# driskai/scenario_gym

Measured on NVIDIA B200. Metric: entity-steps/s, batched rollout+collision, higher is better.
Workload: dtype f64

## Files before the change

### scenario_gym_b200/csrc/sg_common.cuh

```cuda
#pragma once
#include <cuda_runtime.h>
#include <math.h>
#include <stdio.h>
#include <string.h>

#include "sg_device.cuh"
#include "sg_layout.h"

static __constant__ double c_ngon[64][2] = {
#include "sg_ngon.inc"
};

struct Grp {
  int n, s, M, G, W, H, QCAP, bar_id;
  unsigned mask;
  int64_t i, nm;
  double* corners;
  double* actbuf;
  double* rbox;
  unsigned corners_sh, rbox_sh;
  double* tcold;
  double* hcs;
  double* pedbuf;
  float4* pednb;
// ... 637 lines not shown
      group_sync(c);
    }
    const int swapped = *flag;
    ++round;
    if (!swapped) break;
  }
  if (r < c.M) c.posof[c.sid[r]] = (uint16_t)r;
}
SG_DEV void sorted_scatter(const Grp& c) {
  const int p = c.posof[c.s];
  const float k = c.skey[p];
  int np = p;
#pragma unroll
  for (int d = 1; d <= SG_SORT_WIN; ++d) {
    np -= c.skey[p - d] > k ? 1 : 0;
    np += c.skey[p + d] < k ? 1 : 0;
  }
  c.aabb[np] = c.tmpbox[c.s];
  c.sid[np] = (uint16_t)c.s;
  c.posof[c.s] = (uint16_t)np;
}
template <bool VERIFY = false>
SG_DEV void broad_phase_sorted(const Grp& c, int parity) {
  const int r = c.s;
  const float4 mb = c.aabb[r];
  if (VERIFY) {
    const float nx = c.aabb[r + 1].x;
    if (c.posof[c.sid[r]] != r || mb.x > nx) c.sflag[3] = 1;
  }
  if (!(mb.x <= mb.z)) return;
  const float4* nb = c.aabb + r + 1;
  int* acc = c.acc + parity * ACC_N;
  auto push = [&](int d) {
    const int q = atomicAdd(&acc[ACC_QCOUNT], 1);
    if (q < c.QCAP) c.queue[q] = ((uint32_t)c.sid[r] << 16) | (uint32_t)c.sid[r + d];
  };
  uint32_t hits = 0;
#pragma unroll
  for (int dd = 0; dd < SG_SWEEP_WIN; ++dd) {
    const float4 ob = nb[dd];
    SG_AABB_TEST(hits, mb, ob, 1u << dd);
  }
  while (hits) {
    const int dd = __ffs(hits) - 1;
    hits &= hits - 1;
    push(dd + 1);
  }
  for (int d = SG_SWEEP_WIN + 1; r + d < c.M && c.aabb[r + d].x <= mb.z; ++d) {
    const float4 ob = c.aabb[r + d];
    if (mb.x <= ob.z && ob.x <= mb.z && mb.y <= ob.w && ob.y <= mb.w) push(d);
  }
}

SG_DEV void publish_ego_box(const Grp& c) {
  const double eW = c.boxp[c.s], eL = c.boxp[c.G + c.s];
  c.egop[EGO_W] = eW; c.egop[EGO_L] = eL;
  c.egop[EGO_RHW] = 1.0 / (0.5 * eW); c.egop[EGO_RHL] = 1.0 / (0.5 * eL);
}

SG_DEV void unit_norm(double a, double b, double& nn, double& rn) {
  const double s2 = a * a + b * b, d = s2 - 1.0;
  if (fabs(d) < 1e-8) {
    nn = 1.0 + 0.5 * d;
    const double r0 = 2.0 - nn, e = __fma_rn(-nn, r0, 1.0);
    rn = __fma_rn(r0, e, r0);
  } else {
    nn = fast_sqrt(s2);
    rn = fast_rcp(nn);
  }
}

SG_DEV void publish_ego(const Grp& c, bool present, double x, double y, double ec, double es,
                        double vx, double vy) {
  double einv[2];
  {
    double nn, rn;
    unit_norm(es, ec, nn, rn);
    einv[0] = div_r(es, nn, rn);
    einv[1] = div_r(-ec, nn, rn);
  }
  double* E = c.egop;
  E[EGO_X] = x; E[EGO_Y] = y;
  E[EGO_C] = ec; E[EGO_S] = es;
  E[EGO_INV0] = einv[0]; E[EGO_INV1] = einv[1];
  const double hd[2] = {dot2(ec, es, einv[0], einv[1]), dot2(ec, es, ec, es)};
  E[EGO_HD0] = hd[0]; E[EGO_HD1] = hd[1];
  double hinv[2];
  {
    double nn, rn;
    unit_norm(hd[1], hd[0], nn, rn);
    hinv[0] = div_r(hd[1], nn, rn);
    hinv[1] = div_r(-hd[0], nn, rn);
  }
  E[EGO_HINV0] = hinv[0]; E[EGO_HINV1] = hinv[1];
  const double v0 = dot2(vx, vy, einv[0], einv[1]), v1 = dot2(vx, vy, ec, es);
  E[EGO_V0] = v0; E[EGO_V1] = v1;
  E[EGO_VNORM] = fnorm2(v0, v1);
  E[EGO_VLONG] = fabs(dot2(v0, v1, hd[0], hd[1]));
  E[EGO_PRESENT] = present ? 1.0 : 0.0;
}


SG_DEV double qx(unsigned qa, unsigned qs, int k) { return lds_f64(qa + 2u * (unsigned)(k & 3) * qs); }
SG_DEV double qy(unsigned qa, unsigned qs, int k) { return lds_f64(qa + (2u * (unsigned)(k & 3) + 1u) * qs); }
SG_DEV int quad_orientation_sh(unsigned qa, unsigned qs) {
  int s = orient_sign(qx(qa, qs, 0), qy(qa, qs, 0), qx(qa, qs, 1), qy(qa, qs, 1), qx(qa, qs, 2), qy(qa, qs, 2));
  if (s == 0)
    s = orient_sign(qx(qa, qs, 1), qy(qa, qs, 1), qx(qa, qs, 2), qy(qa, qs, 2), qx(qa, qs, 3), qy(qa, qs, 3));
  return s;
}

static __device__ __noinline__ bool line_hits_quad(unsigned qa, unsigned qs, double ax, double ay, double bx,
                                            double by) {
  int pos = 0, neg = 0;
#pragma unroll 1
  for (int m = 0; m < 4; ++m) {
    const int sg = orient_sign(ax, ay, bx, by, qx(qa, qs, m), qy(qa, qs, m));
    pos += sg > 0;
    neg += sg < 0;
  }
  return !(pos == 4 || neg == 4);
}

static __device__ __noinline__ bool quad_hits_centered_rect(unsigned qa, unsigned qs, double a, double b) {
  const int o = quad_orientation_sh(qa, qs);
#pragma unroll 1
  for (int k = 0; k < 4; ++k) {
    const double x0 = qx(qa, qs, k), y0 = qy(qa, qs, k), x1 = qx(qa, qs, k + 1), y1 = qy(qa, qs, k + 1);
    const double dx = x1 - x0, dy = y1 - y0;
    const double py = ((o > 0) == (dx > 0) || dx == 0) ? b : -b;
    const double px = ((o > 0) == (dy > 0) && dy != 0) ? -a : a;
    if (orient_sign(x0, y0, x1, y1, px, py) * o < 0) return false;
  }
  return true;
}

static __device__ __noinline__ bool quad_hits_hsegment(unsigned qa, unsigned qs, double w, double c) {
  const int o = quad_orientation_sh(qa, qs);
#pragma unroll 1
  for (int k = 0; k < 4; ++k) {
    const double x0 = qx(qa, qs, k), y0 = qy(qa, qs, k), x1 = qx(qa, qs, k + 1), y1 = qy(qa, qs, k + 1);
    if (orient_sign(x0, y0, x1, y1, -w, c) * o < 0 && orient_sign(x0, y0, x1, y1, w, c) * o < 0)
      return false;
  }
  return true;
}

static __device__ __noinline__ bool rss_box_hits_segment(unsigned qa, unsigned qs, double x0, double y0,
                                                  double x1, double y1) {
  const Quad q = load_quad_shared(qa, qs);
  return quad_intersects_segment(q, quad_orientation(q), x0, y0, x1, y1);
}

struct RssConst {
  double CLR, RT, MAXA, MINA, r2mina;
};

SG_DEV void rss_ratios(const Grp& c, double x, double y, double* out, int ost) {
  const double* E = c.egop;
  const double eh0 = E[EGO_C], eh1 = E[EGO_S], ei0 = E[EGO_INV0], ei1 = E[EGO_INV1];
  const double dirc = c.hcs[c.s], dirs = c.hcs[c.G + c.s];
  const double bw = c.boxp[c.s], bl = c.boxp[c.G + c.s];
  const double d0 = x - E[EGO_X], d1 = y - E[EGO_Y];
  const double pos0 = dot2(d0, d1, ei0, ei1), pos1 = dot2(d0, d1, eh0, eh1);
  const double hd0 = dot2(dirc, dirs, ei0, ei1), hd1 = dot2(dirc, dirs, eh0, eh1);
  const double eW = E[EGO_W], eL = E[EGO_L];
  const double hn = fnorm2(hd1, hd0), rhn = fast_rcp(hn);
  const double inv0 = div_r(hd1, hn, rhn), inv1 = div_r(-hd0, hn, rhn);
  const double wl_inv = fabs(dot2(bw, bl, inv0, inv1));
  const double wl_dir = fabs(dot2(bw, bl, hd0, hd1));
  const double actual_lat = py_max(1e-6, fabs(pos0) - 0.5 * eW - 0.5 * wl_inv);
  const double actual_long = py_max(1e-6, fabs(pos1) - 0.5 * eL - 0.5 * wl_dir);
  out[2 * ost] = fabs(div_r(actual_lat, 0.5 * eW, E[EGO_RHW]));
  out[3 * ost] = fabs(div_r(actual_long, 0.5 * eL, E[EGO_RHL]));
}

template <bool RATIOS = true>
SG_DEV int rss_hazard(const RssConst& K, const Grp& c, double x, double y, double vx, double vy,
                      uint8_t& state, double* out, int ost) {
  const double* E = c.egop;
  const double eh0 = E[EGO_C], eh1 = E[EGO_S], ei0 = E[EGO_INV0], ei1 = E[EGO_INV1];
  const double dirc = c.hcs[c.s], dirs = c.hcs[c.G + c.s];
  const double bw = c.boxp[c.s], bl = c.boxp[c.G + c.s];
  const double d0 = x - E[EGO_X], d1 = y - E[EGO_Y];
  const double pos0 = dot2(d0, d1, ei0, ei1), pos1 = dot2(d0, d1, eh0, eh1);
  const double hd0 = dot2(dirc, dirs, ei0, ei1), hd1 = dot2(dirc, dirs, eh0, eh1);
  const double v0 = dot2(vx, vy, ei0, ei1), v1 = dot2(vx, vy, eh0, eh1);
  const double eW = E[EGO_W], eL = E[EGO_L];
  const double eHD0 = E[EGO_HD0], eHD1 = E[EGO_HD1];
  double slong;
  {
    const double dp = dot2(eHD0, eHD1, hd0, hd1);
    const double a = fabs(K.MAXA * dp);
    const double hv = dot2(v0, v1, eHD0, eHD1);
    const double rta = K.RT * a;
    const bool ahead = 0.0 > pos1;
    const double vf = ahead ? E[EGO_VNORM] : hv, vr = ahead ? hv : E[EGO_VNORM];
    const double a2 = 2 * a;
    const double vf2a = div_r(vf * vf, a2, fast_rcp(a2));
    const double u = vr + rta;
    const double dd_s = py_max(0, vr * K.RT + py_min(vf2a, 0.5 * a * (K.RT * K.RT)) +
                                      div_r(u * u, 2 * K.MINA, K.r2mina) - vf2a);
    const double v1e = E[EGO_VLONG], av2 = fabs(hv);
    const double u1 = v1e + rta, u2 = av2 + rta;
    const double dd_o = py_max(0, (2 * v1e + rta) * K.RT / 2 + div_r(u1 * u1, 2 * K.MINA, K.r2mina) +
                                      (2 * av2 + rta) * K.RT / 2 + div_r(u2 * u2, 2 * K.MINA, K.r2mina));
    const bool same = dp > 0;
    const bool early = same ? (vr == 0.0) : (np_sign(pos1) == np_sign(v1));
    const double dd = same ? dd_s : dd_o;
    slong = fabs(early ? K.CLR + 0.5 * eL : dd + K.CLR + 0.5 * eL);
  }
  double slat;
  {
    const double k = fabs(dot2(E[EGO_HINV0], E[EGO_HINV1], hd0, hd1));
    const double amax = K.MAXA * k, amin = K.MINA * k;
    const double v = fabs(v0);
    const double den = 2 * amin, rden = fast_rcp(den);
    const double w = K.RT * amax, u = v + w;
    const double dl = py_max(0, 0.5 * K.RT * (2 * v + w) + div_r(u * u, den, rden) -
                                    0.5 * (K.RT * K.RT) * amax - div_r(w * w, den, rden));
    const bool conv = np_sign(-pos0) == np_sign(v0);
    const bool early = conv && v == 0.0;
    const double dd = (conv && !early) ? dl : 0.0;
    slat = fabs(early ? K.CLR + 0.5 * eW : dd + K.CLR + 0.5 * eW);
  }
  out[0] = slat;
  out[ost] = slong;
  if (RATIOS) {
    const double hn = fnorm2(hd1, hd0), rhn = fast_rcp(hn);
    const double inv0 = div_r(hd1, hn, rhn), inv1 = div_r(-hd0, hn, rhn);
    const double wl_inv = fabs(dot2(bw, bl, inv0, inv1));
    const double wl_dir = fabs(dot2(bw, bl, hd0, hd1));
    const double actual_lat = py_max(1e-6, fabs(pos0) - 0.5 * eW - 0.5 * wl_inv);
    const double actual_long = py_max(1e-6, fabs(pos1) - 0.5 * eL - 0.5 * wl_dir);
    out[2 * ost] = fabs(div_r(actual_lat, 0.5 * eW, E[EGO_RHW]));
    out[3 * ost] = fabs(div_r(actual_long, 0.5 * eL, E[EGO_RHL]));
  }
  if ((state >> 2) & 3) return SG_RSS_FOUND;
  double box[8];
#pragma unroll
  for (int q = 0; q < 4; ++q) {
    const double c0 = c.corners[(2 * q) * c.G + c.s] - E[EGO_X];
    const double c1 = c.corners[(2 * q + 1) * c.G + c.s] - E[EGO_Y];
    box[2 * q] = dot2(c0, c1, ei0, ei1);
    box[2 * q + 1] = dot2(c0, c1, eh0, eh1);
  }
  double* rbp = c.rbox + c.s;
#pragma unroll
  for (int q = 0; q < 8; ++q) rbp[q * c.G] = box[q];
  const unsigned rb = c.rbox_sh + (unsigned)c.s * 8u, st = (unsigned)c.G * 8u;
  const double bxmin = min2(min2(box[0], box[2]), min2(box[4], box[6]));
  const double bxmax = max2(max2(box[0], box[2]), max2(box[4], box[6]));
  const double bymin = min2(min2(box[1], box[3]), min2(box[5], box[7]));
  const double bymax = max2(max2(box[1], box[3]), max2(box[5], box[7]));
  bool inter = false;
  if (!(bxmin > slat || bxmax < -slat || bymin > slong || bymax < -slong)) {
    bool corner_in = false;
#pragma unroll
    for (int q = 0; q < 4; ++q)
      corner_in = corner_in || (fabs(box[2 * q]) <= slat && fabs(box[2 * q + 1]) <= slong);
    inter = corner_in || quad_hits_centered_rect(rb, st, slat, slong);
  }
  if (inter) {
    const int marker = state & 3;
    if (marker == 1) { state |= 2 << 2; return SG_RSS_UNSAFE_LONGITUDINAL; }
    if (marker == 2) { state |= 1 << 2; return SG_RSS_UNSAFE_LATERAL; }
    const double ed[2] = {eW, eL};
    double inv[2];
    inverse_direction(ed, inv);
    const double lhs = fabs(fabs(pos0) - fabs(dot2(pos0, pos1, ed[0], ed[1]))) / slat;
    const double rhs = fabs(fabs(pos1 - dot2(pos0, pos1, inv[0], inv[1])) / slong);
    if (lhs > rhs) { state |= 2 << 2; return SG_RSS_UNSAFE_LONGITUDINAL; }
    state |= 1 << 2;
    return SG_RSS_UNSAFE_LATERAL;
  }
  const double L100 = 100 * slong, W100 = 100 * slat;
  bool lat = false, lon = false;
  if (!(bxmin > slat || bxmax < -slat || bymin > L100 || bymax < -L100)) {
    if (bymax < L100 && bymin > -L100) {
      int pos1 = 0, neg1 = 0, pos2 = 0, neg2 = 0;
      bool unsure = false;
#pragma unroll
      for (int q = 0; q < 4; ++q) {
        const double pp = L100 * box[2 * q], rr = slat * box[2 * q + 1];
        const double d1 = pp - rr, d2 = pp + rr, tol = 4e-16 * (fabs(pp) + fabs(rr));
        unsure = unsure || !(fabs(d1) > tol) || !(fabs(d2) > tol);
        pos1 += d1 > 0; neg1 += d1 < 0;
        pos2 += d2 > 0; neg2 += d2 < 0;
      }
      if (unsure)
        lat = line_hits_quad(rb, st, slat, L100, -slat, 100 * -slong) ||
              line_hits_quad(rb, st, -slat, L100, slat, 100 * -slong);
      else
        lat = !(pos1 == 4 || neg1 == 4) || !(pos2 == 4 || neg2 == 4);
    } else
      lat = rss_box_hits_segment(rb, st, slat, L100, -slat, 100 * -slong) ||
            rss_box_hits_segment(rb, st, -slat, L100, slat, 100 * -slong);
  }
  if (!(bxmin > W100 || bxmax < -W100)) {
    if (bxmin > -W100 && bxmax < W100) {
      lon = (bymin <= slong && slong <= bymax) || (bymin <= -slong && -slong <= bymax);
    } else {
      if (!(bymin > slong || bymax < slong)) lon = quad_hits_hsegment(rb, st, W100, slong);
      if (!lon && !(bymin > -slong || bymax < -slong)) lon = quad_hits_hsegment(rb, st, W100, -slong);
    }
  }
  if (lat && lon) return SG_RSS_BOTH;
  if (lat) { state = (uint8_t)((state & ~3) | 1); return SG_RSS_LATERAL; }
  if (lon) { state = (uint8_t)((state & ~3) | 2); return SG_RSS_LONGITUDINAL; }
  return SG_RSS_SAFE;
}

#ifdef SG_FLAT_BOXES
static __device__ __noinline__ bool flat_pair_meets(unsigned pa, unsigned pb, unsigned qs) {
#pragma unroll 1
  for (int i = 0; i < 4; ++i) {
    const double ax = qx(pa, qs, i), ay = qy(pa, qs, i), bx = qx(pa, qs, i + 1), by = qy(pa, qs, i + 1);
#pragma unroll 1
    for (int j = 0; j < 4; ++j)
      if (segments_meet(ax, ay, bx, by, qx(pb, qs, j), qy(pb, qs, j), qx(pb, qs, j + 1), qy(pb, qs, j + 1))) return true;
  }
  return false;
}
#endif

static __device__ __noinline__ bool pair_collides(unsigned csh, const int8_t* orient, int G, int a, int b) {
  const unsigned qs = (unsigned)G * 8u;
  unsigned pa = csh + (unsigned)a * 8u, pb = csh + (unsigned)b * 8u;
  bool same = true;
#pragma unroll 1
  for (unsigned f = 0; f < 8; ++f) same = same && (lds_f64(pa + f * qs) == lds_f64(pb + f * qs));
  if (same) return false;
  int oa = orient[a], ob = orient[b];
#ifdef SG_FLAT_BOXES
  if (oa == 0 && ob == 0) return flat_pair_meets(pa, pb, qs);
#endif
#pragma unroll 1
  for (int pass = 0; pass < 2; ++pass) {
#pragma unroll 1
    for (int k = 0; k < 4; ++k) {
      const double ax = qx(pa, qs, k), ay = qy(pa, qs, k), bx = qx(pa, qs, k + 1), by = qy(pa, qs, k + 1);
      bool sep = true;
#ifdef SG_FLAT_BOXES
      int want = -oa;
#pragma unroll 1
      for (int m = 0; m < 4 && sep; ++m) {
        const int sg = orient_sign(ax, ay, bx, by, qx(pb, qs, m), qy(pb, qs, m));
        if (want == 0) want = sg;
        sep = sg != 0 && sg == want;
      }
#else
#pragma unroll 1
      for (int m = 0; m < 4 && sep; ++m)
        sep = orient_sign(ax, ay, bx, by, qx(pb, qs, m), qy(pb, qs, m)) * oa < 0;
#endif
      if (sep) return false;
    }
    const unsigned tp = pa; pa = pb; pb = tp;
    const int to = oa; oa = ob; ob = to;
  }
  return true;
}

struct PairSink {
  int* acc;
  uint32_t* bits;
  uint32_t* ego_now;
  uint32_t* rows;
  int W, ego_slot, first_slot;
};
SG_DEV PairSink make_sink(int features, uint32_t* coll_mask, const Grp& c, int ego_slot, int first_slot,
                          int parity) {
  PairSink k;
  k.acc = c.acc + parity * ACC_N;
  k.bits = c.bits + parity * c.W;
  k.ego_now = c.ego_now;
  k.rows = (features & SG_FEAT_COLL_MATRIX) ? coll_mask + (int64_t)c.n * c.M * c.W : nullptr;
  k.W = c.W; k.ego_slot = ego_slot; k.first_slot = first_slot;
  return k;
}

static __device__ __noinline__ void commit_pair(PairSink k, int a, int b) {
  const int lo = min(a, b), hi = max(a, b);
  atomicAdd(&k.acc[ACC_NPAIRS], 1);
  atomicMin(&k.acc[ACC_FIRST_PAIR], (lo << 16) | hi);
  if (lo == k.first_slot || hi == k.first_slot) k.acc[ACC_FIRST_HIT] = 1;
  atomicOr(&k.bits[lo >> 5], 1u << (lo & 31));
  atomicOr(&k.bits[hi >> 5], 1u << (hi & 31));
  if (lo == k.ego_slot) atomicOr(&k.ego_now[hi >> 5], 1u << (hi & 31));
  if (hi == k.ego_slot) atomicOr(&k.ego_now[lo >> 5], 1u << (lo & 31));
  if (k.rows) {
    atomicOr(&k.rows[(int64_t)lo * k.W + (hi >> 5)], 1u << (hi & 31));
    atomicOr(&k.rows[(int64_t)hi * k.W + (lo >> 5)], 1u << (lo & 31));
  }
}

SG_DEV int sat_classify(const double* A, const double* B) {
  const double e1ax = A[2] - A[0], e1ay = A[3] - A[1], e2ax = A[0] - A[6], e2ay = A[1] - A[7];
  const double e1bx = B[2] - B[0], e1by = B[3] - B[1], e2bx = B[0] - B[6], e2by = B[1] - B[7];
  const double dx = (B[0] + B[4]) - (A[0] + A[4]), dy = (B[1] + B[5]) - (A[1] + A[5]);
  const double scale = fabs(A[0]) + fabs(A[1]) + fabs(B[0]) + fabs(B[1]) + fabs(e1ax) + fabs(e1ay) + fabs(e2ax) +
                       fabs(e2ay) + fabs(e1bx) + fabs(e1by) + fabs(e2bx) + fabs(e2by);
  const double rel = 1e-9 * scale;
  bool apart = false, inside = true;
#define SG_SAT_AXIS(ax, ay)                                                                             \
  {                                                                                                     \
    const double gap = fabs(dx * (ax) + dy * (ay)) -                                                    \
                       (fabs(e1ax * (ax) + e1ay * (ay)) + fabs(e2ax * (ax) + e2ay * (ay)) +             \
                        fabs(e1bx * (ax) + e1by * (ay)) + fabs(e2bx * (ax) + e2by * (ay)));             \
    const double tol = rel * (fabs(ax) + fabs(ay));                                                     \
    apart = apart || gap > tol;                                                                         \
    inside = inside && gap < -tol;                                                                      \
  }
  SG_SAT_AXIS(e1ax, e1ay)
  SG_SAT_AXIS(e2ax, e2ay)
  SG_SAT_AXIS(e1bx, e1by)
  SG_SAT_AXIS(e2bx, e2by)
#undef SG_SAT_AXIS
  if (!(fabs(dx) + fabs(dy) > rel)) return 0;
  return apart ? -1 : (inside ? 1 : 0);
}

struct Obb {
  double cx, cy, ux, uy, vx, vy;
};
SG_DEV int sat_classify_obb(const Obb& A, const Obb& B) {
  const double dx = B.cx - A.cx, dy = B.cy - A.cy;
  const double scale = fabs(A.cx) + fabs(A.cy) + fabs(B.cx) + fabs(B.cy) + fabs(A.ux) + fabs(A.uy) + fabs(A.vx) +
                       fabs(A.vy) + fabs(B.ux) + fabs(B.uy) + fabs(B.vx) + fabs(B.vy);
  const double rel = 1e-9 * scale;
  bool apart = false, inside = true;
#define SG_OBB_AXIS(ax, ay)                                                                              \
  {                                                                                                     \
    const double gap = fabs(dx * (ax) + dy * (ay)) -                                                    \
                       (fabs(A.ux * (ax) + A.uy * (ay)) + fabs(A.vx * (ax) + A.vy * (ay)) +             \
                        fabs(B.ux * (ax) + B.uy * (ay)) + fabs(B.vx * (ax) + B.vy * (ay)));             \
    const double tol = rel * (fabs(ax) + fabs(ay));                                                     \
    apart = apart || gap > tol;                                                                         \
    inside = inside && gap < -tol;                                                                      \
  }
  SG_OBB_AXIS(A.ux, A.uy)
  SG_OBB_AXIS(A.vx, A.vy)
  SG_OBB_AXIS(B.ux, B.uy)
  SG_OBB_AXIS(B.vx, B.vy)
#undef SG_OBB_AXIS
  if (!(fabs(dx) + fabs(dy) > rel)) return 0;
  return apart ? -1 : (inside ? 1 : 0);
}

SG_DEV void record_pair(const PairSink& k, unsigned corners_sh, const int8_t* orient, int G, int a, int b) {
  if (pair_collides(corners_sh, orient, G, a, b)) commit_pair(k, a, b);
}

static __device__ __noinline__ void decide_pair(PairSink k, const double* corners, unsigned corners_sh,
                                                const int8_t* orient, int G, int a, int b) {
  double qa[8], qb[8];
#pragma unroll
  for (int f = 0; f < 8; ++f) { qa[f] = corners[f * G + a]; qb[f] = corners[f * G + b]; }
  const int v = sat_classify(qa, qb);
// ... 231 lines not shown
```

### scenario_gym_b200/csrc/sg_vehicle.cuh

```cuda
#pragma once
#include "sg_common.cuh"
#include "sg_internal.h"
#include "sg_pcg.cuh"

SG_DEV void cp_async4(unsigned smem_addr, const void* gsrc) {
  asm volatile("cp.async.ca.shared.global [%0], [%1], 4;" ::"r"(smem_addr), "l"(gsrc) : "memory");
}

template <bool RSS, int MC>
struct VehLayout {
  static constexpr GroupLayout value = make_layout(MC > 0 ? MC : 64, false, RSS, true, false);
};
template <bool RSS, int MAXT, int MINB, bool SORTED, bool LEAN = false, int ACT = ACT_F64, int MC = 0>
__global__ void __launch_bounds__(MAXT, MINB)
sg_vehicle_kernel(SgScene sc, SgParams p, SgState st, SgInputs in, int n_ticks, GroupLayout Lrt, SgRngDev rng) {
  extern __shared__ __align__(16) unsigned char smem[];
  const GroupLayout L = MC > 0 ? VehLayout<RSS, MC>::value : Lrt;
  const int G = L.G, M = MC > 0 ? MC : sc.n_slots, W = L.W;
  const int gpb = blockDim.x / G;
  const int gl = threadIdx.x / G;
  const int s = threadIdx.x - gl * G;
  const int n = blockIdx.x * gpb + gl;
  if (gl >= gpb || n >= sc.n_scenarios) return;
  Grp c;
// ... 33 lines not shown
        tc[2 * G] = st.safe_ratio[i]; tc[3 * G] = st.safe_ratio[nm + i];
      }
    }
    if (s == 0) {
      double* U = c.cold_d;
      U[COLD_T0] = st.t[n]; U[COLD_PT0] = st.prev_t[n];
      U[COLD_LEN] = sc.length[n];
      const int64_t er = sc.traj_off[(int64_t)n * M + ego_slot];
      U[COLD_OX] = __ldg(sc.traj_rows + er * 7 + 1);
      U[COLD_OY] = __ldg(sc.traj_rows + er * 7 + 2);
      U[COLD_R2MINA] = 1.0 / (2 * p.rss_min_long_accel);
    }
  }
  int tick = st.tick[n];
  bool done = st.done[n] != 0;
  load_cold(st, c, n, s, W, ego_slot);
  if (RSS && s == ego_slot) publish_ego_box(c);
  if (SORTED) sorted_setup(c);
  int sort_round = 0;
  group_sync(c);

  int limit = n_ticks < 0 ? p.max_ticks : n_ticks;
  if (limit > in.n_action_ticks) limit = in.n_action_ticks;
  int parity = 0;
  const int tick0 = tick;
  double* ab = c.actbuf + s;
  const unsigned ab_sh = (unsigned)__cvta_generic_to_shared(ab);
  const double* act = in.actions + c.i;
  const float* act32 = in.actions_f32 + c.i;
  unsigned long long* rq = (unsigned long long*)c.actbuf + s;
  if (ACT == ACT_RNG) {
    if (live && limit > 0) {
#pragma unroll 1
      for (int cc = 0; cc < 2; ++cc) {
        const sg_u128 q = sg_rng_slot_state(rng, cc, c.i + (int64_t)sc.scenario_base * M);
        rq[(2 * cc) * G] = (unsigned long long)q;
        rq[(2 * cc + 1) * G] = (unsigned long long)(q >> 64);
      }
    }
  } else if (ACT == ACT_F32) {
    if (live && limit > 0 && (!done || in.step_done)) { cp_async4(ab_sh, act32); cp_async4(ab_sh + G * 8, act32 + c.nm); }
    cp_async_commit();
  } else {
    if (live && limit > 0 && (!done || in.step_done)) { cp_async8(ab_sh, act); cp_async8(ab_sh + G * 8, act + c.nm); }
    cp_async_commit();
  }

  double* const corners0 = c.corners;
  const unsigned corners_sh0 = c.corners_sh;
  for (int k = 0; k < limit && (!done || in.step_done); ++k) {
    if (LEAN && lag) {
      c.corners = corners0 + parity * 8 * G;
      c.corners_sh = corners_sh0 + (unsigned)(parity * 8 * G * 8);
    }
    const double* U = c.cold_d;
    const double t = U[COLD_T0 + parity];
    const double next_t = t + p.timestep;
    const double dt = next_t - t;
    if (ACT != ACT_RNG) cp_async_wait_all();
    if (live && present) {
      double a_in, s_in;
      if (ACT == ACT_RNG) {
        const sg_u128 A = sg_u128_make(rng.a_hi, rng.a_lo), Cc = sg_u128_make(rng.c_hi, rng.c_lo);
        unsigned long long lo = rq[0], hi = rq[G];
        a_in = rng.low[0] + rng.scale[0] * sg_pcg_double(hi, lo);
        sg_u128 q = A * sg_u128_make(hi, lo) + Cc;
        rq[0] = (unsigned long long)q; rq[G] = (unsigned long long)(q >> 64);
        lo = rq[2 * G]; hi = rq[3 * G];
        s_in = rng.low[1] + rng.scale[1] * sg_pcg_double(hi, lo);
        q = A * sg_u128_make(hi, lo) + Cc;
        rq[2 * G] = (unsigned long long)q; rq[3 * G] = (unsigned long long)(q >> 64);
      } else if (ACT == ACT_F32) {
        a_in = (double)*(const float*)(ab + parity * 2 * G);
        s_in = (double)*(const float*)(ab + parity * 2 * G + G);
      } else {
        a_in = ab[parity * 2 * G];
        s_in = ab[parity * 2 * G + G];
      }
      const double accel = clipd(a_in, -p.veh_max_accel, p.veh_max_accel);
      const double steer = clipd(s_in, -p.veh_max_steer, p.veh_max_steer);
      const double dx = speed * cs, dy = speed * sn;
      const double tn = fabs(steer) <= 0.78 ? tan_small(steer) : tan_lib(steer);
      const double dh = div_r(speed * tn, c.boxp[G + s], tc[5 * G]);
      const double nx = x + dx * dt, ny = y + dy * dt, nh = h + dh * dt;
      double ns = speed + accel * dt;
      if (!p.veh_allow_reverse) ns = ns < 0.0 ? 0.0 : ns;
      if (p.veh_max_speed == p.veh_max_speed) ns = ns > p.veh_max_speed ? p.veh_max_speed : ns;
      speed = ns;
      const double rdt = fast_rcp(dt);
      const double ex = nx - x, ey = ny - y;
      vx = div_r(ex, dt, rdt); vy = div_r(ey, dt, rdt);
      tc[4 * G] = div_r(nh - h, dt, rdt);
      dist += fnorm2(ex, ey);
      x = nx; y = ny; h = nh;
      sincos_fast(h, sn, cs);
    }
    if (ACT == ACT_F64) {
      if (live && k + 1 < limit) {
        act += 2 * c.nm;
        cp_async8(ab_sh + (parity ^ 1) * 2 * G * 8, act);
        cp_async8(ab_sh + ((parity ^ 1) * 2 * G + G) * 8, act + c.nm);
      }
      cp_async_commit();
    } else if (ACT == ACT_F32) {
      if (live && k + 1 < limit) {
        act32 += 2 * c.nm;
        cp_async4(ab_sh + (parity ^ 1) * 2 * G * 8, act32);
        cp_async4(ab_sh + ((parity ^ 1) * 2 * G + G) * 8, act32 + c.nm);
      }
      cp_async_commit();
    }
    tick += 1;
    if (!LEAN && st.trace_cap > 0 && tick < st.trace_cap && s < M) {
      const int64_t i = c.i, nm = c.nm;
      st.trace_present[(int64_t)tick * nm + i] = present;
      double* tp = st.trace_pose + (int64_t)tick * 6 * nm + i;
      tp[0] = x; tp[nm] = y; tp[2 * nm] = st.pose[2 * nm + i]; tp[3 * nm] = h;
      tp[4 * nm] = st.pose[4 * nm + i]; tp[5 * nm] = st.pose[5 * nm + i];
      if (s == 0) st.trace_t[(int64_t)tick * sc.n_scenarios + n] = next_t;
    }
    if (s < M) {
      if (need_coll || feat_rss)
        publish_box<RSS, SORTED>(c, present, x, y, cs, sn, orient_hint, U[COLD_OX], U[COLD_OY]);
      if (!LEAN && matrix) {
        uint32_t* row = st.coll_mask + ((int64_t)n * M + s) * W;
        for (int w = 0; w < W; ++w) row[w] = 0;
      }
    }
    if (RSS && feat_rss && s == ego_slot) publish_ego(c, present, x, y, cs, sn, vx, vy);
    if (s == 0) {
      c.cold_d[COLD_T0 + (parity ^ 1)] = next_t;
      c.cold_d[COLD_PT0 + (parity ^ 1)] = t;
    }
    group_sync(c);
    bool resort = false;
    if (SORTED && need_coll) {
      resort = c.sflag[3] != 0;
      if (!resort) {
        if (s < M) sorted_scatter(c);
        group_sync(c);
      }
    }
    if (LEAN && lag && k > 0)
      lagged_epilogue(p, st, c, n + sc.scenario_base, s, W, G, ego_slot, parity ^ 1, tick - 1, t);
    if (live && present) {
      if (RSS && feat_rss) {
        rss_last = SG_RSS_NONE;
        rss_evald = false;
        if (next_t != 0.0 && s != ego_slot && c.egop[EGO_PRESENT] != 0.0) {
          RssConst KR;
          KR.CLR = p.rss_min_safe_clearance; KR.RT = p.rss_response_time;
          KR.MAXA = p.rss_max_long_accel; KR.MINA = p.rss_min_long_accel;
          KR.r2mina = c.cold_d[COLD_R2MINA];
          rss_last = (uint8_t)rss_hazard<!LEAN>(KR, c, x, y, vx, vy, rss_state, tc, G);
          rss_evald = true;
          const int found = (rss_state >> 2) & 3;
          if (found) atomicOr(&c.acc[parity * ACC_N + ACC_RSS], found == 2 ? 1 : 2);
        }
      }
      if (need_coll && !SORTED) broad_phase(c, parity);
    }
    if (SORTED && need_coll && !resort && s < M) broad_phase_sorted<true>(c, parity);
    group_sync(c);
    if (SORTED && need_coll && (resort || c.sflag[3] != 0)) {
      group_sync(c);
      if (s == 0) { c.sflag[3] = 0; c.acc[parity * ACC_N + ACC_QCOUNT] = 0; }
      if (s < M) { c.aabb[s] = c.tmpbox[s]; c.sid[s] = (uint16_t)s; }
      group_sync(c);
      sort_positions(c, sort_round);
      group_sync(c);
      if (s < M) broad_phase_sorted<false>(c, parity);
      group_sync(c);
    }
    if (LEAN && lag) {
      narrow_phase_lagged(p, st, c, s, G, ego_slot, first_slot, parity, live && present);
      if (c.acc[parity * ACC_N + ACC_QCOUNT] > c.QCAP) group_sync(c);
      const double ta = c.cold_d[COLD_T0 + (parity ^ 1)], dta = ta - c.cold_d[COLD_PT0 + (parity ^ 1)];
      done = (p.terminal & SG_TERM_MAX_LENGTH) && (ta + dta > c.cold_d[COLD_LEN]);
      if (s == ego_slot && (p.features & SG_FEAT_EGO_METRICS)) {
        double* m = c.cold_d;
        const double sp = fast_sqrt(vx * vx + vy * vy);
        const double w = ta > 0.0 ? div_r(m[COLD_AVG_T], ta, fast_rcp(ta)) : m[COLD_AVG_T] / ta;
        m[COLD_AVG] += (1.0 - w) * (sp - m[COLD_AVG]);
        m[COLD_AVG_T] = ta;
        m[COLD_MAX] = fmax(sp, m[COLD_MAX]);
        m[COLD_EGOD] = dist;
      }
    } else {
      done = finish_tick<true>(p, st, c, n + sc.scenario_base, s, W, G, ego_slot, first_slot, parity, tick,
                         c.cold_d[COLD_T0 + (parity ^ 1)], c.cold_d[COLD_T0 + (parity ^ 1)] - c.cold_d[COLD_PT0 + (parity ^ 1)],
                         c.cold_d[COLD_LEN], live, live && present, collided, vx, vy, 0.0, dist);
    }
    parity ^= 1;
  }
  if (LEAN && lag && tick > tick0) {
    group_sync(c);
    lagged_epilogue(p, st, c, n + sc.scenario_base, s, W, G, ego_slot, parity ^ 1, tick, c.cold_d[COLD_T0 + parity]);
    if (live && ((c.bits[s >> 5] >> (s & 31)) & 1)) collided = 1;
  }

  if (RSS && LEAN && live && present && rss_evald) rss_ratios(c, x, y, tc, G);
  if (live) {
    const int64_t i = c.i, nm = c.nm;
    st.pose[i] = x; st.pose[nm + i] = y; st.pose[3 * nm + i] = h;
    st.vel[i] = vx; st.vel[nm + i] = vy; st.vel[3 * nm + i] = tc[4 * G];
    if (tick > tick0 && present) { st.vel[2 * nm + i] = 0.0; st.vel[4 * nm + i] = 0.0; st.vel[5 * nm + i] = 0.0; }
    st.dist[i] = dist;
    st.speed[i] = speed;
    st.collided[i] = collided;
    if (RSS) {
      st.rss_state[i] = rss_state; st.rss_last[i] = rss_last;
      st.safe_dist[i] = tc[0]; st.safe_dist[nm + i] = tc[G];
      st.safe_ratio[i] = tc[2 * G]; st.safe_ratio[nm + i] = tc[3 * G];
    }
  }
  if (s == 0) {
    st.t[n] = c.cold_d[COLD_T0 + parity]; st.prev_t[n] = c.cold_d[COLD_PT0 + parity];
    st.tick[n] = tick; st.done[n] = done;
  }
  store_cold(st, c, n, s, W, ego_slot);
}

template <bool RSS>
static cudaError_t launch_vehicle_t(int n_scen, cudaStream_t s, const SgScene& sc, const SgParams& p,
                                    const SgState& st, const SgInputs& in, const SgRngDev& rng, int act,
                                    int n_ticks, const GroupLayout& L) {
  void (*kern)(SgScene, SgParams, SgState, SgInputs, int, GroupLayout, SgRngDev);
  int threads;
  const bool lean = sgi_vehicle_lean(p, st);
  if (!lean && act != ACT_F64) return cudaErrorNotSupported;
#define SG_VEH_PICK(T, B, S)                                                                   \
  (!lean ? sg_vehicle_kernel<RSS, T, B, S, false, ACT_F64>                                     \
         : act == ACT_RNG ? sg_vehicle_kernel<RSS, T, B, S, true, ACT_RNG>                     \
         : act == ACT_F32 ? sg_vehicle_kernel<RSS, T, B, S, true, ACT_F32>                     \
                          : sg_vehicle_kernel<RSS, T, B, S, true, ACT_F64>)
#define SG_VEH_PICK_M(T, B, S, MC_)                                                            \
  (act == ACT_RNG ? sg_vehicle_kernel<RSS, T, B, S, true, ACT_RNG, MC_>                        \
                  : sg_vehicle_kernel<RSS, T, B, S, true, ACT_F64, MC_>)
  const int M = sc.n_slots;
  const bool spec = lean && (act == ACT_RNG || act == ACT_F64);
  if (L.G <= SG_VEH_THREADS) {
    kern = (spec && M == 64) ? SG_VEH_PICK_M(SG_VEH_THREADS, SG_VEH_MINB, false, 64)
         : (spec && M == 128) ? SG_VEH_PICK_M(SG_VEH_THREADS, SG_VEH_MINB, false, 128)
                              : SG_VEH_PICK(SG_VEH_THREADS, SG_VEH_MINB, false);
    threads = SG_VEH_THREADS;
  } else if (L.G <= SG_THREADS) {
    kern = (spec && M == 256 && L.sorted) ? SG_VEH_PICK_M(SG_THREADS, 2, true, 256)
         : L.sorted ? SG_VEH_PICK(SG_THREADS, 2, true) : SG_VEH_PICK(SG_THREADS, 2, false);
    threads = SG_THREADS;
  }
  else { kern = L.sorted ? SG_VEH_PICK(1024, 1, true) : SG_VEH_PICK(1024, 1, false); threads = L.G; }
#undef SG_VEH_PICK
#undef SG_VEH_PICK_M
  const int gpb = threads / L.G;
  const int blocks = (n_scen + gpb - 1) / gpb;
  const size_t smem = (size_t)gpb * L.bytes;
  if (smem > 48 * 1024) {
    cudaError_t err = cudaFuncSetAttribute(kern, cudaFuncAttributeMaxDynamicSharedMemorySize, (int)smem);
    if (err != cudaSuccess) return err;
  }
  kern<<<blocks, threads, smem, s>>>(sc, p, st, in, n_ticks, L, rng);
  return cudaGetLastError();
}
```

Baseline: 17.22 billion.

## Add analytic separating-axis fast path for RSS geometry with noinline fallback

For the sorted vehicle kernel, the RSS hazard check first tries a closed-form separating-axis test on the oriented box against the safety rectangle and the lateral and longitudinal bands, with tolerance margins. It falls back to an out-of-line geometry stage that computes the rotated box in shared memory and flags which exact tests to run. The non-sorted path also gains an interval pre-test before the per-corner sign loop. The aim is to cut per-entity arithmetic, register pressure and divergence in RSS evaluation, at the cost of a noinline call on the fallback and a possible mismatch with the exact result near the tolerance edges.

```diff
diff --git a/scenario_gym_b200/csrc/sg_common.cuh b/scenario_gym_b200/csrc/sg_common.cuh
--- a/scenario_gym_b200/csrc/sg_common.cuh
+++ b/scenario_gym_b200/csrc/sg_common.cuh
@@ -813,6 +813,75 @@
   return quad_intersects_segment(q, quad_orientation(q), x0, y0, x1, y1);
 }
 
+enum : unsigned {
+  RSS_GEO_RECT = 1u,
+  RSS_GEO_LINES = 2u,
+  RSS_GEO_SEGS = 4u,
+  RSS_GEO_HSEG_P = 8u,
+  RSS_GEO_HSEG_M = 16u,
+  RSS_GEO_LAT = 32u,
+  RSS_GEO_LON = 64u,
+  RSS_GEO_INTER = 128u,
+};
+static __device__ __noinline__ unsigned rss_geometry_stage(unsigned ca, unsigned rb, unsigned st, unsigned ea,
+                                                           double slat, double slong) {
+  const double ex = lds_f64(ea + EGO_X * 8u), ey = lds_f64(ea + EGO_Y * 8u);
+  const double eh0 = lds_f64(ea + EGO_C * 8u), eh1 = lds_f64(ea + EGO_S * 8u);
+  const double ei0 = lds_f64(ea + EGO_INV0 * 8u), ei1 = lds_f64(ea + EGO_INV1 * 8u);
+  double* const box = (double*)__cvta_shared_to_generic(rb);
+  const unsigned G = st / 8u;
+  bool corner_in = false;
+#pragma unroll 1
+  for (unsigned q = 0; q < 4; ++q) {
+    const double c0 = lds_f64(ca + 2u * q * st) - ex;
+    const double c1 = lds_f64(ca + (2u * q + 1u) * st) - ey;
+    const double b0 = dot2(c0, c1, ei0, ei1), b1 = dot2(c0, c1, eh0, eh1);
+    box[2u * q * G] = b0;
+    box[(2u * q + 1u) * G] = b1;
+    corner_in = corner_in || (fabs(b0) <= slat && fabs(b1) <= slong);
+  }
+#define SG_BX(q) box[2u * (q) * G]
+#define SG_BY(q) box[(2u * (q) + 1u) * G]
+  const double bxmin = min2(min2(SG_BX(0), SG_BX(1)), min2(SG_BX(2), SG_BX(3)));
+  const double bxmax = max2(max2(SG_BX(0), SG_BX(1)), max2(SG_BX(2), SG_BX(3)));
+  const double bymin = min2(min2(SG_BY(0), SG_BY(1)), min2(SG_BY(2), SG_BY(3)));
+  const double bymax = max2(max2(SG_BY(0), SG_BY(1)), max2(SG_BY(2), SG_BY(3)));
+  const bool near = !(bxmin > slat || bxmax < -slat || bymin > slong || bymax < -slong);
+  if (near && corner_in) return RSS_GEO_INTER;
+  unsigned todo = near ? RSS_GEO_RECT : 0u;
+  {
+    const double L100 = 100 * slong, W100 = 100 * slat;
+    if (!(bxmin > slat || bxmax < -slat || bymin > L100 || bymax < -L100)) {
+      if (bymax < L100 && bymin > -L100) {
+        int pos1 = 0, neg1 = 0, pos2 = 0, neg2 = 0;
+        bool unsure = false;
+#pragma unroll 1
+        for (unsigned q = 0; q < 4; ++q) {
+          const double pp = L100 * SG_BX(q), rr = slat * SG_BY(q);
+          const double d1 = pp - rr, d2 = pp + rr, tol = 4e-16 * (fabs(pp) + fabs(rr));
+          unsure = unsure || !(fabs(d1) > tol) || !(fabs(d2) > tol);
+          pos1 += d1 > 0; neg1 += d1 < 0;
+          pos2 += d2 > 0; neg2 += d2 < 0;
+        }
+        if (unsure) todo |= RSS_GEO_LINES;
+        else if (!(pos1 == 4 || neg1 == 4) || !(pos2 == 4 || neg2 == 4)) todo |= RSS_GEO_LAT;
+      } else
+        todo |= RSS_GEO_SEGS;
+    }
+    if (!(bxmin > W100 || bxmax < -W100)) {
+      if (bxmin > -W100 && bxmax < W100) {
+        if ((bymin <= slong && slong <= bymax) || (bymin <= -slong && -slong <= bymax)) todo |= RSS_GEO_LON;
+      } else {
+        if (!(bymin > slong || bymax < slong)) todo |= RSS_GEO_HSEG_P;
+        if (!(bymin > -slong || bymax < -slong)) todo |= RSS_GEO_HSEG_M;
+      }
+    }
+  }
+#undef SG_BX
+#undef SG_BY
+  return todo;
+}
+
 struct RssConst {
   double CLR, RT, MAXA, MINA, r2mina;
 };
@@ -836,7 +905,7 @@
   out[3 * ost] = fabs(div_r(actual_long, 0.5 * eL, E[EGO_RHL]));
 }
 
-template <bool RATIOS = true>
+template <bool RATIOS = true, bool BAND = false>
 SG_DEV int rss_hazard(const RssConst& K, const Grp& c, double x, double y, double vx, double vy,
                       uint8_t& state, double* out, int ost) {
   const double* E = c.egop;
@@ -898,31 +967,141 @@
     out[3 * ost] = fabs(div_r(actual_long, 0.5 * eL, E[EGO_RHL]));
   }
   if ((state >> 2) & 3) return SG_RSS_FOUND;
-  double box[8];
+  if (!BAND) {
+    double box[8];
 #pragma unroll
-  for (int q = 0; q < 4; ++q) {
-    const double c0 = c.corners[(2 * q) * c.G + c.s] - E[EGO_X];
-    const double c1 = c.corners[(2 * q + 1) * c.G + c.s] - E[EGO_Y];
-    box[2 * q] = dot2(c0, c1, ei0, ei1);
-    box[2 * q + 1] = dot2(c0, c1, eh0, eh1);
-  }
-  double* rbp = c.rbox + c.s;
+    for (int q = 0; q < 4; ++q) {
+      const double c0 = c.corners[(2 * q) * c.G + c.s] - E[EGO_X];
+      const double c1 = c.corners[(2 * q + 1) * c.G + c.s] - E[EGO_Y];
+      box[2 * q] = dot2(c0, c1, ei0, ei1);
+      box[2 * q + 1] = dot2(c0, c1, eh0, eh1);
+    }
+    double* rbp = c.rbox + c.s;
 #pragma unroll
-  for (int q = 0; q < 8; ++q) rbp[q * c.G] = box[q];
-  const unsigned rb = c.rbox_sh + (unsigned)c.s * 8u, st = (unsigned)c.G * 8u;
-  const double bxmin = min2(min2(box[0], box[2]), min2(box[4], box[6]));
-  const double bxmax = max2(max2(box[0], box[2]), max2(box[4], box[6]));
-  const double bymin = min2(min2(box[1], box[3]), min2(box[5], box[7]));
-  const double bymax = max2(max2(box[1], box[3]), max2(box[5], box[7]));
-  bool inter = false;
-  if (!(bxmin > slat || bxmax < -slat || bymin > slong || bymax < -slong)) {
-    bool corner_in = false;
+    for (int q = 0; q < 8; ++q) rbp[q * c.G] = box[q];
+    const unsigned rb = c.rbox_sh + (unsigned)c.s * 8u, st = (unsigned)c.G * 8u;
+    const double bxmin = min2(min2(box[0], box[2]), min2(box[4], box[6]));
+    const double bxmax = max2(max2(box[0], box[2]), max2(box[4], box[6]));
+    const double bymin = min2(min2(box[1], box[3]), min2(box[5], box[7]));
+    const double bymax = max2(max2(box[1], box[3]), max2(box[5], box[7]));
+    bool inter = false;
+    if (!(bxmin > slat || bxmax < -slat || bymin > slong || bymax < -slong)) {
+      bool corner_in = false;
 #pragma unroll
-    for (int q = 0; q < 4; ++q)
-      corner_in = corner_in || (fabs(box[2 * q]) <= slat && fabs(box[2 * q + 1]) <= slong);
-    inter = corner_in || quad_hits_centered_rect(rb, st, slat, slong);
-  }
-  if (inter) {
+      for (int q = 0; q < 4; ++q)
+        corner_in = corner_in || (fabs(box[2 * q]) <= slat && fabs(box[2 * q + 1]) <= slong);
+      inter = corner_in || quad_hits_centered_rect(rb, st, slat, slong);
+    }
+    if (inter) {
+      const int marker = state & 3;
+      if (marker == 1) { state |= 2 << 2; return SG_RSS_UNSAFE_LONGITUDINAL; }
+      if (marker == 2) { state |= 1 << 2; return SG_RSS_UNSAFE_LATERAL; }
+      const double ed[2] = {eW, eL};
+      double inv[2];
+      inverse_direction(ed, inv);
+      const double lhs = fabs(fabs(pos0) - fabs(dot2(pos0, pos1, ed[0], ed[1]))) / slat;
+      const double rhs = fabs(fabs(pos1 - dot2(pos0, pos1, inv[0], inv[1])) / slong);
+      if (lhs > rhs) { state |= 2 << 2; return SG_RSS_UNSAFE_LONGITUDINAL; }
+      state |= 1 << 2;
+      return SG_RSS_UNSAFE_LATERAL;
+    }
+    const double L100 = 100 * slong, W100 = 100 * slat;
+    bool lat = false, lon = false;
+    if (!(bxmin > slat || bxmax < -slat || bymin > L100 || bymax < -L100)) {
+      if (bymax < L100 && bymin > -L100) {
+        const double a0 = L100 * bxmin, a1 = L100 * bxmax, b0 = slat * bymin, b1 = slat * bymax;
+        const double tl = 4e-16 * ((fabs(a0) + fabs(a1)) + (fabs(b0) + fabs(b1)));
+        if (!((a0 - b1 > tl || a1 - b0 < -tl) && (a0 + b0 > tl || a1 + b1 < -tl))) {
+          int pos1 = 0, neg1 = 0, pos2 = 0, neg2 = 0;
+          bool unsure = false;
+#pragma unroll
+          for (int q = 0; q < 4; ++q) {
+            const double pp = L100 * box[2 * q], rr = slat * box[2 * q + 1];
+            const double d1 = pp - rr, d2 = pp + rr, tol = 4e-16 * (fabs(pp) + fabs(rr));
+            unsure = unsure || !(fabs(d1) > tol) || !(fabs(d2) > tol);
+            pos1 += d1 > 0; neg1 += d1 < 0;
+            pos2 += d2 > 0; neg2 += d2 < 0;
+          }
+          if (unsure)
+            lat = line_hits_quad(rb, st, slat, L100, -slat, 100 * -slong) ||
+                  line_hits_quad(rb, st, -slat, L100, slat, 100 * -slong);
+          else
+            lat = !(pos1 == 4 || neg1 == 4) || !(pos2 == 4 || neg2 == 4);
+        }
+      } else
+        lat = rss_box_hits_segment(rb, st, slat, L100, -slat, 100 * -slong) ||
+              rss_box_hits_segment(rb, st, -slat, L100, slat, 100 * -slong);
+    }
+    if (!(bxmin > W100 || bxmax < -W100)) {
+      if (bxmin > -W100 && bxmax < W100) {
+        lon = (bymin <= slong && slong <= bymax) || (bymin <= -slong && -slong <= bymax);
+      } else {
+        if (!(bymin > slong || bymax < slong)) lon = quad_hits_hsegment(rb, st, W100, slong);
+        if (!lon && !(bymin > -slong || bymax < -slong)) lon = quad_hits_hsegment(rb, st, W100, -slong);
+      }
+    }
+    if (lat && lon) return SG_RSS_BOTH;
+    if (lat) { state = (uint8_t)((state & ~3) | 1); return SG_RSS_LATERAL; }
+    if (lon) { state = (uint8_t)((state & ~3) | 2); return SG_RSS_LONGITUDINAL; }
+    return SG_RSS_SAFE;
+  }
+  unsigned geo = 8u;
+  const double bcx = c.boxp[2 * c.G + c.s], bcy = c.boxp[3 * c.G + c.s];
+  const double hl = 0.5 * fabs(bl), hw = 0.5 * fabs(bw);
+  const double ah0 = fabs(hd0), ah1 = fabs(hd1);
+  const double del = 1e-9 * (((fabs(x) + fabs(y)) + (fabs(E[EGO_X]) + fabs(E[EGO_Y]))) +
+                             ((fabs(bl) + fabs(bw)) + (fabs(bcx) + fabs(bcy))));
+  if (hl > del && hw > del && ah0 + ah1 < 1.5 && del > 1e-150 && slat > 1e-100 && slong > 1e-100 &&
+      del + slat + slong < 1e50) {
+    const double c0 = pos0 + (bcx * hd0 - bcy * hd1), c1 = pos1 + (bcx * hd1 + bcy * hd0);
+    const double ac0 = fabs(c0), ac1 = fabs(c1);
+    const double ex = hl * ah0 + hw * ah1, ey = hl * ah1 + hw * ah0;
+    const double gx = ac0 - (ex + slat), gy = ac1 - (ey + slong);
+    bool apart = gx > del || gy > del;
+    if (!apart) {
+      const double mh = del * (ah0 + ah1);
+      const double gu = fabs(hd0 * c0 + hd1 * c1) - (hl + (ah0 * slat + ah1 * slong));
+      const double gv = fabs(hd0 * c1 - hd1 * c0) - (hw + (ah1 * slat + ah0 * slong));
+      if (gx < -del && gy < -del && gu < -mh && gv < -mh) geo = 1u;
+      apart = gu > mh || gv > mh;
+    }
+    if (apart) {
+      const double L100 = 100 * slong, W100 = 100 * slat;
+      const double ml = del * (L100 + slat);
+      const double P = L100 * c0, Q = slat * c1;
+      const double ea = L100 * ex + slat * ey;
+      bool lat_t = false, lat_f = ac1 - ey - L100 > del || (fabs(P - Q) - ea > ml && fabs(P + Q) - ea > ml);
+      if (!lat_f) {
+        const double A = L100 * hd0, B = slat * hd1, C = L100 * hd1, D = slat * hd0;
+        const double g1 = fabs(P - Q) - (hl * fabs(A - B) + hw * fabs(C + D));
+        const double g2 = fabs(P + Q) - (hl * fabs(A + B) + hw * fabs(C - D));
+        lat_t = ac1 + ey - L100 < -del && (g1 < -ml || g2 < -ml);
+        lat_f = g1 > ml && g2 > ml;
+      }
+      const double gp = fabs(c1 - slong) - ey, gm = fabs(c1 + slong) - ey;
+      const bool lon_t = ac0 + ex - W100 < -del && (gp < -del || gm < -del);
+      const bool lon_f = ac0 - ex - W100 > del || (gp > del && gm > del);
+      if ((lat_t || lat_f) && (lon_t || lon_f)) geo = (lat_t ? 2u : 0u) | (lon_t ? 4u : 0u);
+    }
+  }
+  if (geo == 8u) {
+    const unsigned rb = c.rbox_sh + (unsigned)c.s * 8u, st = (unsigned)c.G * 8u;
+    const unsigned todo = rss_geometry_stage(c.corners_sh + (unsigned)c.s * 8u, rb, st,
+                                             (unsigned)__cvta_generic_to_shared(E), slat, slong);
+    if ((todo & RSS_GEO_INTER) || ((todo & RSS_GEO_RECT) && quad_hits_centered_rect(rb, st, slat, slong))) {
+      geo = 1u;
+    } else {
+      const double L100 = 100 * slong, W100 = 100 * slat;
+      const bool lat = (todo & RSS_GEO_LAT) ||
+                       ((todo & RSS_GEO_LINES) && (line_hits_quad(rb, st, slat, L100, -slat, 100 * -slong) ||
+                                                   line_hits_quad(rb, st, -slat, L100, slat, 100 * -slong))) ||
+                       ((todo & RSS_GEO_SEGS) && (rss_box_hits_segment(rb, st, slat, L100, -slat, 100 * -slong) ||
+                                                  rss_box_hits_segment(rb, st, -slat, L100, slat, 100 * -slong)));
+      const bool lon = (todo & RSS_GEO_LON) || ((todo & RSS_GEO_HSEG_P) && quad_hits_hsegment(rb, st, W100, slong)) ||
+                       ((todo & RSS_GEO_HSEG_M) && quad_hits_hsegment(rb, st, W100, -slong));
+      geo = (lat ? 2u : 0u) | (lon ? 4u : 0u);
+    }
+  }  if (geo & 1u) {
     const int marker = state & 3;
     if (marker == 1) { state |= 2 << 2; return SG_RSS_UNSAFE_LONGITUDINAL; }
     if (marker == 2) { state |= 1 << 2; return SG_RSS_UNSAFE_LATERAL; }
@@ -935,37 +1114,7 @@
     state |= 1 << 2;
     return SG_RSS_UNSAFE_LATERAL;
   }
-  const double L100 = 100 * slong, W100 = 100 * slat;
-  bool lat = false, lon = false;
-  if (!(bxmin > slat || bxmax < -slat || bymin > L100 || bymax < -L100)) {
-    if (bymax < L100 && bymin > -L100) {
-      int pos1 = 0, neg1 = 0, pos2 = 0, neg2 = 0;
-      bool unsure = false;
-#pragma unroll
-      for (int q = 0; q < 4; ++q) {
-        const double pp = L100 * box[2 * q], rr = slat * box[2 * q + 1];
-        const double d1 = pp - rr, d2 = pp + rr, tol = 4e-16 * (fabs(pp) + fabs(rr));
-        unsure = unsure || !(fabs(d1) > tol) || !(fabs(d2) > tol);
-        pos1 += d1 > 0; neg1 += d1 < 0;
-        pos2 += d2 > 0; neg2 += d2 < 0;
-      }
-      if (unsure)
-        lat = line_hits_quad(rb, st, slat, L100, -slat, 100 * -slong) ||
-              line_hits_quad(rb, st, -slat, L100, slat, 100 * -slong);
-      else
-        lat = !(pos1 == 4 || neg1 == 4) || !(pos2 == 4 || neg2 == 4);
-    } else
-      lat = rss_box_hits_segment(rb, st, slat, L100, -slat, 100 * -slong) ||
-            rss_box_hits_segment(rb, st, -slat, L100, slat, 100 * -slong);
-  }
-  if (!(bxmin > W100 || bxmax < -W100)) {
-    if (bxmin > -W100 && bxmax < W100) {
-      lon = (bymin <= slong && slong <= bymax) || (bymin <= -slong && -slong <= bymax);
-    } else {
-      if (!(bymin > slong || bymax < slong)) lon = quad_hits_hsegment(rb, st, W100, slong);
-      if (!lon && !(bymin > -slong || bymax < -slong)) lon = quad_hits_hsegment(rb, st, W100, -slong);
-    }
-  }
+  const bool lat = (geo & 2u) != 0, lon = (geo & 4u) != 0;
   if (lat && lon) return SG_RSS_BOTH;
   if (lat) { state = (uint8_t)((state & ~3) | 1); return SG_RSS_LATERAL; }
   if (lon) { state = (uint8_t)((state & ~3) | 2); return SG_RSS_LONGITUDINAL; }
diff --git a/scenario_gym_b200/csrc/sg_vehicle.cuh b/scenario_gym_b200/csrc/sg_vehicle.cuh
--- a/scenario_gym_b200/csrc/sg_vehicle.cuh
+++ b/scenario_gym_b200/csrc/sg_vehicle.cuh
@@ -209,7 +209,7 @@
           KR.CLR = p.rss_min_safe_clearance; KR.RT = p.rss_response_time;
           KR.MAXA = p.rss_max_long_accel; KR.MINA = p.rss_min_long_accel;
           KR.r2mina = c.cold_d[COLD_R2MINA];
-          rss_last = (uint8_t)rss_hazard<!LEAN>(KR, c, x, y, vx, vy, rss_state, tc, G);
+          rss_last = (uint8_t)rss_hazard<!LEAN, SORTED>(KR, c, x, y, vx, vy, rss_state, tc, G);
           rss_evald = true;
           const int found = (rss_state >> 2) & 3;
           if (found) atomicOr(&c.acc[parity * ACC_N + ACC_RSS], found == 2 ? 1 : 2);
```

Measured after the change: 17.26 billion, median of 6. No clear change (+0.2%).
